# ICLDisco/parsec

Measured on AMD Instinct MI355X. Metric: GFLOP/s (whole node) tiled Cholesky N=80k, higher is better.
Workload: dtype fp64; 1 GPU; model=tiled_cholesky_dpotrf, N=80000, tile=4096, parallelism=dtd-tile-p1q1, chore_gemm=rocblas, gpu=True

## Files before the change

### src/kernels_hip.cpp

```cpp
#include "kernels_hip.hpp"

#include "kernels.hpp"

namespace pa {

typedef double f64x4 __attribute__((ext_vector_type(4)));

#define BM 128
#define BN 128
#define BKD 16


__device__ __forceinline__ int xcd_swizzle(int id, int nwg) {
  int q = nwg >> 3, r = nwg & 7;
  int xcd = id & 7, pos = id >> 3;
  return (xcd < r ? xcd * (q + 1) : r * (q + 1) + (xcd - r) * q) + pos;
}

__device__ __forceinline__ void tri_decode(int id, int& i, int& j) {
  i = 0;
  while (id > i) { i++; id -= i; }
  j = id;
}

__device__ __forceinline__ void block_decode(bool tri, int nbx, int& bx,
                                             int& by) {
  int id = xcd_swizzle(blockIdx.x, gridDim.x);
  if (tri) {
    tri_decode(id, bx, by);
  } else {
    bx = id % nbx;
    by = id / nbx;
  }
}

__device__ __forceinline__ void mfma_ktile(f64x4 (&acc)[2][4],
                                           const double* ap, const double* bp,
                                           int ld) {
#pragma unroll
  for (int kk = 0; kk < BKD; kk += 4) {
    double a[2], b[4];
#pragma unroll
    for (int f = 0; f < 2; f++) a[f] = ap[kk * ld + f * 16];
#pragma unroll
    for (int f = 0; f < 4; f++) b[f] = bp[kk * ld + f * 16];
#pragma unroll
    for (int i = 0; i < 2; i++)
#pragma unroll
      for (int j = 0; j < 4; j++)
        acc[i][j] =
            __builtin_amdgcn_mfma_f64_16x16x4f64(a[i], b[j], acc[i][j], 0, 0, 0);
  }
}

__device__ __forceinline__ void write_c(const f64x4 (&acc)[2][4], double* C,
                                        int ldc, int row0, int col0, int m,
                                        int n, bool checked, bool store) {
#pragma unroll
  for (int j = 0; j < 4; j++) {
    int col = col0 + j * 16;
    if (checked && col >= n) continue;
    double* cp = C + (size_t)col * ldc;
#pragma unroll
    for (int i = 0; i < 2; i++) {
#pragma unroll
      for (int e = 0; e < 4; e++) {
        int row = row0 + i * 16 + e * 4;
        if (checked && row >= m) continue;
        if (store) cp[row] = acc[i][j][e];
        else cp[row] -= acc[i][j][e];
      }
    }
  }
}

template <bool TRI>
__launch_bounds__(512)
__global__ void k_dgemm_nt_v2(int m, int n, int k, const double* __restrict__ A,
                              int lda, const double* __restrict__ B, int ldb,
                              double* __restrict__ C, int ldc, int nbx) {
  extern __shared__ __attribute__((aligned(16))) char smem[];
  constexpr int LDT = 129;
  double* As = (double*)smem;
  double* Bs = As + 2 * BKD * LDT;
  const int tid = threadIdx.x;
  const int wave = tid >> 6, lane = tid & 63;
  const int wr = wave >> 1, wc = wave & 1;
  int bx, by;
  block_decode(TRI, nbx, bx, by);
  const int bm0 = bx * BM, bn0 = by * BN;
  const int ksub = lane >> 4, r16 = lane & 15;

  f64x4 acc[2][4] = {};

  auto stage = [&](int buf, int k0) {
    double* as = As + buf * BKD * LDT;
    double* bs = Bs + buf * BKD * LDT;
#pragma unroll
    for (int x = 0; x < BM * BKD; x += 512) {
      int xi = x + tid;
      int i = xi & (BM - 1), kk = xi >> 7;
      int gi = bm0 + i, gk = k0 + kk;
      as[kk * LDT + i] = (gi < m && gk < k) ? A[(size_t)gk * lda + gi] : 0.0;
    }
#pragma unroll
    for (int x = 0; x < BN * BKD; x += 512) {
      int xi = x + tid;
      int j = xi & (BN - 1), kk = xi >> 7;
      int gj = bn0 + j, gk = k0 + kk;
      bs[kk * LDT + j] = (gj < n && gk < k) ? B[(size_t)gk * ldb + gj] : 0.0;
    }
  };

  stage(0, 0);
  __syncthreads();
  const int ntiles = (k + BKD - 1) / BKD;
  for (int t = 0; t < ntiles; t++) {
    if (t + 1 < ntiles) stage((t + 1) & 1, (t + 1) * BKD);
    mfma_ktile(acc, As + ((t & 1) * BKD + ksub) * LDT + wr * 32 + r16,
               Bs + ((t & 1) * BKD + ksub) * LDT + wc * 64 + r16, LDT);
    __syncthreads();
  }
  write_c(acc, C, ldc, bm0 + wr * 32 + ksub, bn0 + wc * 64 + r16, m, n,
          true, false);
}

enum { V3_GEMM = 0, V3_SYRK = 1, V3_TRMM = 2 };

template <int KIND>
__launch_bounds__(512)
__global__ void k_dgemm_nt_v3(int m, int n, int k, const double* __restrict__ A,
                              int lda, const double* __restrict__ B, int ldb,
                              double* __restrict__ C, int ldc, int nbx) {
  extern __shared__ __attribute__((aligned(16))) char smem[];
  double* As = (double*)smem;
  double* Bs = As + 2 * BKD * BM;
  const int tid = threadIdx.x;
  const int wave = tid >> 6, lane = tid & 63;
  const int wr = wave >> 1, wc = wave & 1;
  int bx, by;
  if (KIND == V3_TRMM) {
    const int nby = n / BN;
    const int xcd = blockIdx.x & 7, pos = blockIdx.x >> 3;
    const int round = pos / nbx;
    const int rank = round * 8 + ((round & 1) ? 7 - xcd : xcd);
    if (rank >= nby) return;
    bx = pos - round * nbx;
    by = nby - 1 - rank;
  } else {
    block_decode(KIND == V3_SYRK, nbx, bx, by);
  }
  const int bm0 = bx * BM, bn0 = by * BN;
  const int ksub = lane >> 4, r16 = lane & 15;
  const int kend = KIND == V3_TRMM ? (bn0 + BN < k ? bn0 + BN : k) : k;

  f64x4 acc[2][4] = {};

  auto stage = [&](int buf, int k0) {
#pragma unroll
    for (int p = 0; p < 2; p++) {
      int krow = wave * 2 + p;
      const double* srcA = A + (size_t)(k0 + krow) * lda + bm0 + 2 * lane;
      double* dstA = As + buf * BKD * BM + krow * BM;
      __builtin_amdgcn_global_load_lds(
          (const __attribute__((address_space(1))) unsigned int*)srcA,
          (__attribute__((address_space(3))) unsigned int*)dstA, 16, 0, 0);
      const double* srcB = B + (size_t)(k0 + krow) * ldb + bn0 + 2 * lane;
      double* dstB = Bs + buf * BKD * BN + krow * BN;
      __builtin_amdgcn_global_load_lds(
          (const __attribute__((address_space(1))) unsigned int*)srcB,
          (__attribute__((address_space(3))) unsigned int*)dstB, 16, 0, 0);
    }
  };

  stage(0, 0);
  __syncthreads();
  const int ntiles = kend / BKD;
  for (int t = 0; t < ntiles; t++) {
    if (t + 1 < ntiles) stage((t + 1) & 1, (t + 1) * BKD);
    mfma_ktile(acc, As + ((t & 1) * BKD + ksub) * BM + wr * 32 + r16,
               Bs + ((t & 1) * BKD + ksub) * BN + wc * 64 + r16, BM);
    __syncthreads();
  }
  write_c(acc, C, ldc, bm0 + wr * 32 + ksub, bn0 + wc * 64 + r16, m, n,
          false, KIND == V3_TRMM);
}

template <auto Kern, typename... Args>
static void launch_lds(int grid, int block, size_t lds, hipStream_t stream,
                       Args... args) {
  static const bool raised = [lds] {
    PA_HIP_CHECK(hipFuncSetAttribute(
        (const void*)Kern, hipFuncAttributeMaxDynamicSharedMemorySize, lds));
    return true;
  }();
  (void)raised;
  hipLaunchKernelGGL(Kern, dim3(grid), dim3(block), lds, stream, args...);
}

constexpr size_t LDS_V2 = 4 * BKD * 129 * 8;
constexpr size_t LDS_V3 = 2 * BKD * (BM + BN) * 8;

static bool full_tiles(int m, int n, int k, int lda, int ldb) {
  return m % BM == 0 && n % BN == 0 && k % BKD == 0 && lda % 2 == 0 &&
         ldb % 2 == 0;
}

void launch_dgemm_nt(int m, int n, int k, const double* A, int lda,
                     const double* B, int ldb, double* C, int ldc,
                     hipStream_t stream) {
  const int nbx = (m + BM - 1) / BM, nby = (n + BN - 1) / BN;
  if (full_tiles(m, n, k, lda, ldb))
    launch_lds<k_dgemm_nt_v3<V3_GEMM>>(nbx * nby, 512, LDS_V3, stream, m, n, k,
                                       A, lda, B, ldb, C, ldc, nbx);
  else
    launch_lds<k_dgemm_nt_v2<false>>(nbx * nby, 512, LDS_V2, stream, m, n, k,
                                     A, lda, B, ldb, C, ldc, nbx);
}

void launch_dsyrk_ln(int n, int k, const double* A, int lda, double* C,
                     int ldc, hipStream_t stream) {
  const int ntb = (n + BM - 1) / BM;
  const int nblocks = ntb * (ntb + 1) / 2;
  if (full_tiles(n, n, k, lda, lda))
    launch_lds<k_dgemm_nt_v3<V3_SYRK>>(nblocks, 512, LDS_V3, stream, n, n, k,
                                       A, lda, A, lda, C, ldc, 0);
  else
    launch_lds<k_dgemm_nt_v2<true>>(nblocks, 512, LDS_V2, stream, n, n, k, A,
                                    lda, A, lda, C, ldc, 0);
}

void launch_dtrmm_rlt(int m, int n, const double* B, int ldb, const double* W,
                      int ldw, double* X, int ldx, hipStream_t stream) {
  PA_CHECK(m > 0 && n > 0 && full_tiles(m, n, n, ldb, ldw),
           "dtrmm_rlt needs full 128x128 blocks and even ld, got %d x %d, "
           "ldb %d, ldw %d", m, n, ldb, ldw);
  PA_CHECK(ldb >= m && ldx >= m && ldw >= n);
  const int nbx = m / BM, nby = n / BN;
  launch_lds<k_dgemm_nt_v3<V3_TRMM>>(8 * ((nby + 7) / 8) * nbx, 512, LDS_V3,
                                     stream, m, n, n, B, ldb, W, ldw, X, ldx,
                                     nbx);
}

void gpu_gemm_hip(Task& t, GpuTaskCtx& g) {
  const TileArgs& a = t.arg<TileArgs>();
  launch_dgemm_nt(a.m, a.n, a.k, (const double*)t.dev_ptr[0], a.ld,
                  (const double*)t.dev_ptr[1], a.ld, (double*)t.dev_ptr[2],
                  a.ld, g.stream);
}

__global__ void __launch_bounds__(256) k_potf2_mfma(double* A, int n, int ld) {
  extern __shared__ __attribute__((aligned(16))) char smem[];
  constexpr int LDP = 129;
  double* S = (double*)smem;
  double* dinv = S + 128 * LDP;
  const int tid = threadIdx.x;
  const int lane = tid & 63;
  const int wave = tid >> 6;
  for (int x = tid; x < n * n; x += 256) {
    int j = x / n, i = x - j * n;
    if (i >= j) S[j * LDP + i] = A[(size_t)j * ld + i];
  }
  __syncthreads();
  for (int jb = 0; jb < n; jb += 16) {
    const int jbe = jb + 16 < n ? jb + 16 : n;
    for (int j = jb; j < jbe; j++) {
      if (tid == 0) {
        double d = S[j * LDP + j];
        S[j * LDP + j] = d = sqrt(d);
        *dinv = 1.0 / d;
      }
      __syncthreads();
      for (int i = j + 1 + tid; i < n; i += 256) S[j * LDP + i] *= *dinv;
      __syncthreads();
      for (int c = j + 1 + wave; c < jbe; c += 4) {
        double ljc = S[j * LDP + c];
        for (int i = c + lane; i < n; i += 64)
          S[c * LDP + i] -= S[j * LDP + i] * ljc;
      }
      __syncthreads();
    }
    const int t0 = jbe;
    const int nt = (n - t0 + 15) >> 4;
    if (nt > 0) {
      const int ntiles = nt * (nt + 1) / 2;
      const int r16 = lane & 15, g4 = lane >> 4;
      for (int idx = wave; idx < ntiles; idx += 4) {
        int ti, tj;
        tri_decode(idx, ti, tj);
        const int ro = t0 + ti * 16, co = t0 + tj * 16;
        const int arow = ro + r16, brow = co + r16;
        f64x4 acc;
#pragma unroll
        for (int e = 0; e < 4; e++) {
          int r = ro + 4 * e + g4, c = co + r16;
          acc[e] = (r < n && c < n) ? S[c * LDP + r] : 0.0;
        }
#pragma unroll
        for (int kk = 0; kk < 16; kk += 4) {
          int kcol = jb + kk + g4;
          double a = (arow < n) ? -S[kcol * LDP + arow] : 0.0;
          double b = (brow < n) ? S[kcol * LDP + brow] : 0.0;
          acc = __builtin_amdgcn_mfma_f64_16x16x4f64(a, b, acc, 0, 0, 0);
        }
#pragma unroll
        for (int e = 0; e < 4; e++) {
          int r = ro + 4 * e + g4, c = co + r16;
          if (r < n && c < n && r >= c) S[c * LDP + r] = acc[e];
        }
      }
    }
    __syncthreads();
  }
  for (int x = tid; x < n * n; x += 256) {
    int j = x / n, i = x - j * n;
    if (i >= j) A[(size_t)j * ld + i] = S[j * LDP + i];
  }
}

void launch_potf2(double* A, int n, int ld, hipStream_t stream) {
  PA_CHECK(n <= 128);
  launch_lds<k_potf2_mfma>(1, 256, 128 * 129 * 8 + 16, stream, A, n, ld);
}

namespace {

struct DevArray {
  double* p = nullptr;
  size_t bytes;
  explicit DevArray(size_t nelem, const double* host = nullptr)
      : bytes(nelem * 8) {
    PA_HIP_CHECK(hipMalloc(&p, bytes));
    if (host) PA_HIP_CHECK(hipMemcpy(p, host, bytes, hipMemcpyHostToDevice));
  }
  DevArray(const DevArray&) = delete;
  ~DevArray() { PA_HIP_CHECK(hipFree(p)); }
  void download(double* host) {
    PA_HIP_CHECK(hipGetLastError());
    PA_HIP_CHECK(hipMemcpy(host, p, bytes, hipMemcpyDeviceToHost));
  }
};

__global__ void k_bench_fill(double* p, size_t n, uint32_t seed) {
  size_t i = (size_t)blockIdx.x * blockDim.x + threadIdx.x;
  for (; i < n; i += (size_t)gridDim.x * blockDim.x) {
    uint64_t h = (i * 2654435761ull) ^ ((uint64_t)seed * 2246822519ull);
    h ^= h >> 13;
    h *= 0x9E3779B97F4A7C15ull;
    h ^= h >> 32;
    p[i] = (double)(h & 0xFFFFFF) / (double)0x1000000 - 0.5;
  }
}

void bench_fill(DevArray& a, uint32_t seed) {
  hipLaunchKernelGGL(k_bench_fill, dim3(2048), dim3(256), 0, 0, a.p,
                     a.bytes / 8, seed);
}

template <typename F>
double time_launches(int iters, F run) {
  run();
  PA_HIP_CHECK(hipDeviceSynchronize());
  double t0 = now_s();
  for (int i = 0; i < iters; i++) run();
  PA_HIP_CHECK(hipDeviceSynchronize());
  return now_s() - t0;
}

}

void test_dgemm_nt_hip(int m, int n, int k, const double* A, int lda,
                       const double* B, int ldb, double* C, int ldc) {
  DevArray dA((size_t)lda * k, A), dB((size_t)ldb * k, B),
      dC((size_t)ldc * n, C);
  launch_dgemm_nt(m, n, k, dA.p, lda, dB.p, ldb, dC.p, ldc, 0);
  dC.download(C);
}

void test_dsyrk_ln_hip(int n, int k, const double* A, int lda, double* C,
                       int ldc) {
  DevArray dA((size_t)lda * k, A), dC((size_t)ldc * n, C);
  launch_dsyrk_ln(n, k, dA.p, lda, dC.p, ldc, 0);
  dC.download(C);
}

void test_dtrmm_rlt_hip(int m, int n, const double* B, int ldb,
                        const double* W, int ldw, double* X, int ldx) {
  DevArray dB((size_t)ldb * n, B), dW((size_t)ldw * n, W),
      dX((size_t)ldx * n, X);
  launch_dtrmm_rlt(m, n, dB.p, ldb, dW.p, ldw, dX.p, ldx, 0);
  dX.download(X);
}

void test_potf2_hip(double* A, int n) {
  DevArray dA((size_t)n * n, A);
  launch_potf2(dA.p, n, n, 0);
  dA.download(A);
}

double bench_dgemm_hip(int m, int n, int k, int iters) {
  DevArray dA((size_t)m * k), dB((size_t)n * k), dC((size_t)m * n);
  bench_fill(dA, 11);
  bench_fill(dB, 12);
  bench_fill(dC, 13);
  return time_launches(iters, [&] {
    launch_dgemm_nt(m, n, k, dA.p, m, dB.p, n, dC.p, m, 0);
  });
}

double bench_dtrmm_hip(int m, int n, int iters) {
  DevArray dB((size_t)m * n), dW((size_t)n * n), dX((size_t)m * n);
  bench_fill(dB, 11);
  bench_fill(dW, 12);
  for (int c = 1; c < n; c++)
    PA_HIP_CHECK(hipMemsetAsync(dW.p + (size_t)c * n, 0, (size_t)c * 8, 0));
  return time_launches(iters, [&] {
    launch_dtrmm_rlt(m, n, dB.p, m, dW.p, n, dX.p, m, 0);
  });
}

}
```

### src/kernels_hip.hpp

```cpp
#pragma once

#include "device_gpu.hpp"

namespace pa {

void launch_dgemm_nt(int m, int n, int k, const double* A, int lda,
                     const double* B, int ldb, double* C, int ldc,
                     hipStream_t stream);
void launch_dsyrk_ln(int n, int k, const double* A, int lda, double* C,
                     int ldc, hipStream_t stream);
void launch_dtrmm_rlt(int m, int n, const double* B, int ldb, const double* W,
                      int ldw, double* X, int ldx, hipStream_t stream);
void launch_potf2(double* A, int n, int ld, hipStream_t stream);

void gpu_gemm_hip(Task& t, GpuTaskCtx& g);

void test_dgemm_nt_hip(int m, int n, int k, const double* A, int lda,
                       const double* B, int ldb, double* C, int ldc);
void test_dsyrk_ln_hip(int n, int k, const double* A, int lda, double* C,
                       int ldc);
void test_dtrmm_rlt_hip(int m, int n, const double* B, int ldb,
                        const double* W, int ldw, double* X, int ldx);
void test_potf2_hip(double* A, int n);

double bench_dgemm_hip(int m, int n, int k, int iters);
double bench_dtrmm_hip(int m, int n, int iters);

}
```

### src/pybind.cpp

```cpp
#include <pybind11/numpy.h>
#include <pybind11/pybind11.h>
#include <pybind11/stl.h>

#include <chrono>
#include <map>

#include "data.hpp"
#include "device_gpu.hpp"
#include "comm.hpp"
#include "dtd.hpp"
#include "gpu_graph.hpp"
#include "kernels.hpp"
#include "kernels_hip.hpp"
#include "pins.hpp"
#include "profiling.hpp"
#include "runtime.hpp"

namespace pa {
std::string rccl_get_unique_id();
void rccl_set_unique_id(const std::string&);
double bench_dgemm_rocblas(int, int, int, int);
double bench_gemm_bf16(int, int, int, int);
double bench_qr_factor(int, int, int, int, int);
void test_gemm_bf16_hip(int, int, int, const uint16_t*, const uint16_t*,
                        float*);
}

namespace py = pybind11;
using namespace pa;

namespace {

struct PyTaskPayload {
  PyObject* fn;
  int with_data;
};

void py_task_hook(Task& t) {
  const PyTaskPayload& pl = t.arg<PyTaskPayload>();
  void* bufs[MAX_FLOWS] = {};
  if (pl.with_data) {
    for (int i = 0; i < t.nflows; i++) {
      Data* d = t.flows[i].data;
      if (!d) continue;
      if (t.flows[i].mode & ACCESS_IN) {
        bufs[i] = d->pull_to_host();
      } else {
        d->begin_host_overwrite();
        bufs[i] = d->ensure_host();
      }
    }
  }
  py::gil_scoped_acquire gil;
  py::handle fn(pl.fn);
  try {
    if (pl.with_data) {
      py::tuple args(t.nflows);
      for (int i = 0; i < t.nflows; i++) {
        Data* d = t.flows[i].data;
        if (d)
          args[i] = py::memoryview::from_memory(bufs[i], (ssize_t)d->bytes);
        else
          args[i] = py::none();
      }
      fn(*args);
    } else {
      fn();
    }
  } catch (py::error_already_set& e) {
    fprintf(stderr, "[parsec_amd] python task raised: %s\n", e.what());
  }
  for (int i = 0; i < t.nflows && pl.with_data; i++)
    if (t.flows[i].data && (t.flows[i].mode & ACCESS_OUT))
      t.flows[i].data->written_on(false);
}

void py_task_destruct(Task& t) {
  py::gil_scoped_acquire gil;
  Py_XDECREF(t.arg<PyTaskPayload>().fn);
}

TaskClass& py_task_class() {
  static TaskClass tc = [] {
    TaskClass c;
    c.name = "py_task";
    c.kind = TaskKind::CPU;
    c.cpu_hook = py_task_hook;
    c.destruct = py_task_destruct;
    c.id = 100;
    return c;
  }();
  return tc;
}

Context::Options options_from_env(int nworkers, int rank, int world,
                                  std::string comm, int gpu) {
  Context::Options o;
  o.nworkers = nworkers;
  if (rank < 0) {
    const char* r = getenv("RANK");
    const char* w = getenv("WORLD_SIZE");
    o.rank = r ? atoi(r) : 0;
    o.world = w ? atoi(w) : 1;
  } else {
    o.rank = rank;
    o.world = world;
  }
  o.comm = std::move(comm);
  o.gpu_device = gpu;
  return o;
}

}

PYBIND11_MODULE(_core, m) {
  m.doc() = "parsec_amd: MI355X-native task-dataflow runtime (PaRSEC-class)";

  py::class_<Context>(m, "Context")
      .def(py::init([](int nworkers, int rank, int world, std::string comm,
                       int gpu) {
             return new Context(
                 options_from_env(nworkers, rank, world, std::move(comm), gpu));
           }),
           py::arg("nworkers") = -1, py::arg("rank") = -1,
           py::arg("world") = -1, py::arg("comm") = std::string(),
           py::arg("gpu") = -1,
           py::call_guard<py::gil_scoped_release>())
      .def_property_readonly("_handle", [](Context& c) { return (uintptr_t)&c; })
      .def_property_readonly("rank", &Context::rank)
      .def_property_readonly("world", &Context::world)
      .def_property_readonly("nworkers", &Context::nworkers)
      .def_property_readonly("has_gpu", &Context::has_gpu)
      .def("barrier", &Context::barrier,
           py::call_guard<py::gil_scoped_release>())
      .def("gpu_sync", [](Context& c) {
        if (c.gpu()) c.gpu()->sync_all();
      }, py::call_guard<py::gil_scoped_release>())
      .def("gpu_stats", [](Context& c) {
        py::dict d;
        if (c.gpu()) {
          d["tasks"] = c.gpu()->stats.tasks.load();
          d["bytes_h2d"] = c.gpu()->stats.bytes_h2d.load();
          d["bytes_d2h"] = c.gpu()->stats.bytes_d2h.load();
          d["evictions"] = c.gpu()->stats.evictions.load();
          d["bytes_required"] = c.gpu()->stats.bytes_required.load();
        }
        return d;
      })
      .def("send_ctl", [](Context& c, int dst, uint32_t tag, py::bytes b) {
        PA_CHECK(c.comm(), "send_ctl: no comm engine");
        std::string s(b);
        py::gil_scoped_release rel;
        c.comm()->send_ctl(dst, tag, s.data(), s.size());
      }, py::arg("dst"), py::arg("tag"), py::arg("payload"))
      .def("set_ctl_handler", [](Context& c, py::function fn) {
        PA_CHECK(c.comm(), "set_ctl_handler: no comm engine");
        PyObject* f = fn.ptr();
        Py_XINCREF(f);
        c.comm()->set_ctl_handler(
            [f](int src, uint32_t tag, const std::string& pl) {
              py::gil_scoped_acquire gil;
              try {
                py::handle h(f);
                h(src, tag, py::bytes(pl));
              } catch (py::error_already_set& e) {
                fprintf(stderr, "[parsec_amd] ctl handler raised: %s\n",
                        e.what());
              }
            });
      })
      .def("info", [](Context& c) {
        py::dict d;
        for (auto& [k, v] : c.info_all()) d[py::str(k)] = v;
        return d;
      })
      .def("info_set", [](Context& c, std::string k, std::string v) {
        c.info_set(k, v);
      })
      .def("comm_stats", [](Context& c) {
        py::list out;
        if (c.comm()) {
          for (auto& ps : c.comm()->peer_stats()) {
            py::dict d;
            d["sent_msgs"] = ps.sent_msgs.load();
            d["sent_bytes"] = ps.sent_bytes.load();
            d["recv_msgs"] = ps.recv_msgs.load();
            d["recv_bytes"] = ps.recv_bytes.load();
            out.append(d);
          }
        }
        return out;
      })
      .def("counters", [](Context&) {
        auto& c = counters();
        py::dict d;
        d["tasks_executed_cpu"] = c.tasks_executed_cpu.load();
        d["tasks_executed_gpu"] = c.tasks_executed_gpu.load();
        d["tasks_scheduled"] = c.tasks_scheduled.load();
        d["steals"] = c.steals.load();
        d["comm_msgs"] = c.comm_msgs.load();
        d["comm_bytes"] = c.comm_bytes.load();
        d["renames"] = c.renames.load();
        return d;
      });

  py::class_<Data>(m, "Data")
      .def_property_readonly("home_rank", [](Data& d) { return d.home_rank; })
      .def_property_readonly("owner_rank", [](Data& d) { return d.owner_rank; })
      .def_property_readonly("version", [](Data& d) { return d.version; })
      .def_property_readonly("nbytes", [](Data& d) { return d.bytes; });

  py::class_<TiledMatrix>(m, "TiledMatrix")
      .def(py::init<Context*, int64_t, int64_t, int, int, int, int, size_t,
                    bool>(),
           py::arg("ctx"), py::arg("m"), py::arg("n"), py::arg("mb"),
           py::arg("nb"), py::arg("p") = 1, py::arg("q") = 1,
           py::arg("elem_size") = 8, py::arg("sym") = false,
           py::keep_alive<1, 2>())
      .def_property_readonly("_handle", [](TiledMatrix& a) { return (uintptr_t)&a; })
      .def_property_readonly("m", &TiledMatrix::m)
      .def_property_readonly("n", &TiledMatrix::n)
      .def_property_readonly("mt", &TiledMatrix::mt)
      .def_property_readonly("nt", &TiledMatrix::nt)
      .def_property_readonly("mb", &TiledMatrix::mb)
      .def_property_readonly("nb", &TiledMatrix::nb)
      .def("rank_of", &TiledMatrix::rank_of)
      .def("set_kcyclic", &TiledMatrix::set_kcyclic)
      .def("set_rank_table", &TiledMatrix::set_rank_table)
      .def("set_band", &TiledMatrix::set_band)
      .def("in_band", &TiledMatrix::in_band)
      .def("is_local", &TiledMatrix::is_local)
      .def("tile", &TiledMatrix::tile, py::return_value_policy::reference_internal)
      .def("tile_rows", &TiledMatrix::tile_rows)
      .def("tile_cols", &TiledMatrix::tile_cols)
      .def("tile_numpy", [](TiledMatrix& A, int tm, int tn) {
        PA_CHECK(A.is_local(tm, tn), "tile_numpy: tile is not local");
        Data* d = A.tile(tm, tn);
        double* p;
        {
          py::gil_scoped_release rel;
          p = (double*)d->pull_to_host();
        }
        int rows = A.tile_rows(tm), cols = A.tile_cols(tn);
        py::array_t<double> out({rows, cols});
        auto r = out.mutable_unchecked<2>();
        for (int j = 0; j < cols; j++)
          for (int i = 0; i < rows; i++) r(i, j) = p[(size_t)j * A.mb() + i];
        return out;
      })
      .def("tile_numpy_set", [](TiledMatrix& A, int tm, int tn,
                                py::array_t<double> v) {
        PA_CHECK(A.is_local(tm, tn), "tile_numpy_set: tile is not local");
        Data* d = A.tile(tm, tn);
        d->begin_host_overwrite();
        double* p = (double*)d->ensure_host();
        auto r = v.unchecked<2>();
        int rows = A.tile_rows(tm), cols = A.tile_cols(tn);
        PA_CHECK(r.shape(0) == rows && r.shape(1) == cols);
        for (int j = 0; j < cols; j++)
          for (int i = 0; i < rows; i++) p[(size_t)j * A.mb() + i] = r(i, j);
        d->written_on(false);
      })
      .def("tile_bytes", [](TiledMatrix& A, int tm, int tn) {
        PA_CHECK(A.is_local(tm, tn));
        Data* d = A.tile(tm, tn);
        void* p;
        {
          py::gil_scoped_release rel;
          p = d->pull_to_host();
        }
        return py::bytes((const char*)p, d->bytes);
      })
      .def("tile_bytes_set", [](TiledMatrix& A, int tm, int tn, py::bytes b) {
        PA_CHECK(A.is_local(tm, tn));
        Data* d = A.tile(tm, tn);
        d->begin_host_overwrite();
        std::string s(b);
        PA_CHECK(s.size() <= d->bytes);
        memcpy(d->ensure_host(), s.data(), s.size());
        d->written_on(false);
      });

  py::class_<ZoneAlloc>(m, "ZoneAlloc")
      .def(py::init([](size_t bytes) {
             auto* z = new ZoneAlloc();
             z->init(bytes);
             return z;
           }),
           py::arg("bytes"))
      .def("alloc",
           [](ZoneAlloc& z, size_t sz) -> py::object {
             size_t off = z.alloc(sz);
             if (off == ZoneAlloc::NPOS) return py::none();
             return py::int_(off);
           })
      .def("free", &ZoneAlloc::free, py::arg("off"), py::arg("size"))
      .def_property_readonly("in_use", &ZoneAlloc::in_use)
      .def_property_readonly("capacity", &ZoneAlloc::capacity)
      .def_property_readonly("largest_free", &ZoneAlloc::largest_free)
      .def_property_readonly("free_blocks", &ZoneAlloc::free_blocks);

  py::class_<IrregularCollection>(m, "IrregularCollection")
      .def(py::init<Context*>(), py::arg("ctx"), py::keep_alive<1, 2>())
      .def("add", &IrregularCollection::add, py::arg("key"), py::arg("rank"),
           py::arg("bytes"), py::return_value_policy::reference_internal)
      .def("at", &IrregularCollection::at, py::arg("key"),
           py::return_value_policy::reference_internal)
      .def_property_readonly("size", &IrregularCollection::size)
      .def("bytes_get", [](IrregularCollection& c, uint64_t key) {
        Data* d = c.at(key);
        void* p;
        {
          py::gil_scoped_release rel;
          p = d->pull_to_host();
        }
        return py::bytes((const char*)p, d->bytes);
      })
      .def("bytes_set", [](IrregularCollection& c, uint64_t key, py::bytes b) {
        Data* d = c.at(key);
        d->begin_host_overwrite();
        std::string s2(b);
        PA_CHECK(s2.size() <= d->bytes);
        memcpy(d->ensure_host(), s2.data(), s2.size());
        d->written_on(false);
      });

  py::class_<Taskpool>(m, "Taskpool")
      .def("wait_dynamic", &Taskpool::wait_dynamic,
           py::call_guard<py::gil_scoped_release>())
      .def_property_readonly("_handle", [](Taskpool& t) { return (uintptr_t)&t; })
      .def("wait", &Taskpool::wait, py::call_guard<py::gil_scoped_release>())
      .def_property_readonly("pending", &Taskpool::pending)
      .def("on_complete", [](Taskpool& t, py::function fn) {
        auto holder = std::shared_ptr<py::function>(
            new py::function(std::move(fn)), [](py::function* p) {
              py::gil_scoped_acquire gil;
              delete p;
            });
        t.on_complete([holder] {
          py::gil_scoped_acquire gil;
          try {
            (*holder)();
          } catch (py::error_already_set& e) {
            fprintf(stderr, "[parsec_amd] on_complete raised: %s\n", e.what());
          }
        });
      });

  py::class_<Dtd, Taskpool>(m, "Dtd")
      .def(py::init<Context*, std::string>(), py::arg("ctx"),
           py::arg("name") = std::string("dtd"), py::keep_alive<1, 2>())
      .def("insert_py",
           [](Dtd& tp, py::function fn, py::list flows, int priority,
              int rank, bool with_data) {
             PyTaskPayload pl{fn.ptr(), with_data ? 1 : 0};
             Py_XINCREF(pl.fn);
             std::vector<Dtd::FlowSpec> fs;
             for (auto h : flows) {
               auto t2 = h.cast<py::tuple>();
               Dtd::FlowSpec f{t2[0].cast<Data*>(),
                               (AccessMode)t2[1].cast<int>(),
                               Reshape::NONE};
               if (t2.size() > 2) f.reshape = (Reshape)t2[2].cast<int>();
               fs.push_back(f);
             }
             bool local;
             {
               py::gil_scoped_release rel;
               local = tp.insert(&py_task_class(), &pl, sizeof(pl),
                                 fs.data(), (int)fs.size(), priority, rank);
             }
             if (!local) Py_XDECREF(pl.fn);
           },
           py::arg("fn"), py::arg("flows") = py::list(),
           py::arg("priority") = 0, py::arg("rank") = -1,
           py::arg("with_data") = false)
      .def("flush", &Dtd::flush, py::call_guard<py::gil_scoped_release>())
      .def("flush_all", &Dtd::flush_all,
           py::call_guard<py::gil_scoped_release>())
      .def("capture_begin", &Dtd::capture_begin)
      .def("capture_end", &Dtd::capture_end,
           py::call_guard<py::gil_scoped_release>(),
           py::keep_alive<0, 1>());

  py::class_<GpuGraph>(m, "GpuGraph")
      .def("launch", &GpuGraph::launch, py::arg("iters") = 1,
           py::call_guard<py::gil_scoped_release>())
      .def_property_readonly("nodes", &GpuGraph::nodes)
      .def_property_readonly("n_tasks", &GpuGraph::n_tasks);

  m.attr("ACCESS_IN") = (int)ACCESS_IN;
  m.attr("ACCESS_UNTRACKED") = (int)ACCESS_UNTRACKED;
  m.attr("ACCESS_OUT") = (int)ACCESS_OUT;
  m.attr("ACCESS_INOUT") = (int)ACCESS_INOUT;
  m.attr("RESHAPE_TRANSPOSE") = (int)Reshape::TRANSPOSE;
  m.attr("RESHAPE_TO_BF16") = (int)Reshape::TO_BF16;
  m.attr("RESHAPE_FROM_BF16") = (int)Reshape::FROM_BF16;
  m.attr("RESHAPE_TRIL") = (int)Reshape::TRIL;
  m.attr("RESHAPE_TRIU") = (int)Reshape::TRIU;

  m.def("bench_qr_factor", &bench_qr_factor, py::arg("m"), py::arg("k"),
        py::arg("ts_split"), py::arg("iters"), py::arg("mode"),
        py::call_guard<py::gil_scoped_release>());
  m.def("insert_spd_fill", &insert_spd_fill, py::arg("tp"), py::arg("A"),
        py::arg("seed") = 42u, py::call_guard<py::gil_scoped_release>());
  m.def("insert_full_fill", &insert_full_fill, py::arg("tp"), py::arg("A"),
        py::arg("seed") = 42u, py::call_guard<py::gil_scoped_release>());
  m.def("insert_potrf", &insert_potrf, py::arg("tp"), py::arg("A"),
        py::call_guard<py::gil_scoped_release>());
  m.def("insert_getrf_nopiv", &insert_getrf_nopiv, py::arg("tp"),
        py::arg("A"), py::call_guard<py::gil_scoped_release>());
  m.def("insert_geqrf", &insert_geqrf, py::arg("tp"), py::arg("A"),
        py::call_guard<py::gil_scoped_release>());
  m.def("insert_geqrf_bcgs", &insert_geqrf_bcgs, py::arg("tp"),
        py::arg("A"), py::arg("R"), py::call_guard<py::gil_scoped_release>());
  m.def("insert_redistribute", &insert_redistribute, py::arg("tp"),
        py::arg("src"), py::arg("dst"), py::call_guard<py::gil_scoped_release>());
  m.def("insert_reduce_axis", &insert_reduce_axis, py::arg("tp"),
        py::arg("A"), py::arg("R"), py::arg("axis"),
        py::call_guard<py::gil_scoped_release>());
  m.def("insert_band_to_rect", &insert_band_to_rect, py::arg("tp"),
        py::arg("S"), py::arg("D"), py::call_guard<py::gil_scoped_release>());
  m.def("insert_subtile_extract", &insert_subtile_extract, py::arg("tp"),
        py::arg("A"), py::arg("tm"), py::arg("tn"), py::arg("S"),
        py::call_guard<py::gil_scoped_release>());
  m.def("insert_subtile_insert", &insert_subtile_insert, py::arg("tp"),
        py::arg("S"), py::arg("A"), py::arg("tm"), py::arg("tn"),
        py::call_guard<py::gil_scoped_release>());
  m.def("insert_potrs", &insert_potrs, py::arg("tp"), py::arg("A"),
        py::arg("B"), py::call_guard<py::gil_scoped_release>());
  m.def("insert_posv", &insert_posv, py::arg("tp"), py::arg("A"),
        py::arg("B"), py::call_guard<py::gil_scoped_release>());
  m.def("insert_getrs_nopiv", &insert_getrs_nopiv, py::arg("tp"),
        py::arg("A"), py::arg("B"), py::call_guard<py::gil_scoped_release>());
  m.def("insert_gesv_nopiv", &insert_gesv_nopiv, py::arg("tp"),
        py::arg("A"), py::arg("B"), py::call_guard<py::gil_scoped_release>());
  m.def("insert_gels_bcgs", &insert_gels_bcgs, py::arg("tp"), py::arg("A"),
        py::arg("R"), py::arg("B"), py::arg("X"),
        py::call_guard<py::gil_scoped_release>());
  m.def("insert_advise_prefetch", &insert_advise_prefetch, py::arg("tp"),
        py::arg("tile"), py::call_guard<py::gil_scoped_release>());
  m.def("insert_gemm_fp64", &insert_gemm_fp64, py::arg("tp"), py::arg("A"),
        py::arg("B"), py::arg("C"),
        py::call_guard<py::gil_scoped_release>());
  m.def("insert_apply_scale", &insert_apply_scale, py::arg("tp"), py::arg("A"),
        py::arg("alpha"), py::arg("beta"),
        py::call_guard<py::gil_scoped_release>());
  m.def("insert_reduce_sum_tree", &insert_reduce_sum_tree, py::arg("tp"),
        py::arg("A"), py::arg("R"), py::call_guard<py::gil_scoped_release>());
  m.def("insert_reduce_sum", &insert_reduce_sum, py::arg("tp"), py::arg("A"),
        py::arg("R"), py::call_guard<py::gil_scoped_release>());
  m.def("insert_stencil_1d", &insert_stencil_1d, py::arg("tp"),
        py::arg("src"), py::arg("dst"), py::call_guard<py::gil_scoped_release>());
  m.def("insert_panel_fill", &insert_panel_fill, py::arg("tp"), py::arg("A"),
        py::arg("seed") = 42u, py::call_guard<py::gil_scoped_release>());
  m.def("insert_potrf_panel", &insert_potrf_panel, py::arg("tp"),
        py::arg("A"), py::call_guard<py::gil_scoped_release>());
  m.def("insert_fill_bf16", &insert_fill_bf16, py::arg("tp"), py::arg("A"),
        py::arg("seed") = 1u, py::call_guard<py::gil_scoped_release>());
  m.def("insert_gemm_bf16", &insert_gemm_bf16, py::arg("tp"), py::arg("At"),
        py::arg("B"), py::arg("C"), py::call_guard<py::gil_scoped_release>());
  m.def("bench_gemm_bf16", [](int m, int n, int k, int iters) {
    return pa::bench_gemm_bf16(m, n, k, iters);
  }, py::call_guard<py::gil_scoped_release>());
  m.def("gemm_bf16_hip", [](py::array_t<uint16_t> A, py::array_t<uint16_t> B,
                            py::array_t<float> C, int m, int n, int k) {
    pa::test_gemm_bf16_hip(m, n, k, A.data(), B.data(), C.mutable_data());
  });

  m.def("pins_add", [](py::function fn, std::vector<std::string> events) {
    static const std::map<std::string, PinsEv> names = {
        {"exec_begin", PinsEv::EXEC_BEGIN}, {"exec_end", PinsEv::EXEC_END},
        {"schedule", PinsEv::SCHEDULE},     {"complete", PinsEv::COMPLETE},
        {"gpu_submit", PinsEv::GPU_SUBMIT}, {"gpu_retire", PinsEv::GPU_RETIRE},
        {"create", PinsEv::CREATE},
        {"release_deps", PinsEv::RELEASE_DEPS},
        {"stage_in", PinsEv::STAGE_IN},     {"comm_post", PinsEv::COMM_POST},
        {"comm_done", PinsEv::COMM_DONE},   {"steal", PinsEv::STEAL}};
    uint32_t mask = 0;
    for (auto& e : events) {
      auto it = names.find(e);
      if (it == names.end())
        throw std::invalid_argument("unknown PINS event: " + e);
      mask |= 1u << (int)it->second;
    }
    auto keep = std::shared_ptr<py::function>(
        new py::function(std::move(fn)), [](py::function* f) {
          py::gil_scoped_acquire g;
          delete f;
        });
    static const char* evname[] = {"exec_begin", "exec_end",   "schedule",
                                   "complete",   "gpu_submit", "gpu_retire",
                                   "create",     "release_deps", "stage_in",
                                   "comm_post",  "comm_done",  "steal"};
    return Pins::inst().add(
        [keep](PinsEv e, const Task* t, int worker) {
          py::gil_scoped_acquire g;
          (*keep)(evname[(int)e], t ? t->tc->name : std::string(), worker);
        },
        mask);
  });
  m.def("pins_remove", [](int id) { Pins::inst().remove(id); });

  m.def("set_fatal_handler", [](py::function fn) {
    static py::function* g_fn = nullptr;
    if (g_fn) { delete g_fn; }
    g_fn = new py::function(std::move(fn));
    set_fatal_handler(+[](const char* msg) {
      py::gil_scoped_acquire g;
      try { (*reinterpret_cast<py::function*>(g_fn))(msg); } catch (...) {}
    });
  });

  m.def("param_set", &param_set);
  m.def("param_dump", &param_dump);
  m.def("hip_device_count", [] {
    int n = 0;
    if (hipGetDeviceCount(&n) != hipSuccess) n = 0;
    return n;
  });
  m.def("dgemm_nt_hip", [](py::array_t<double> A, py::array_t<double> B,
                           py::array_t<double> C, int m, int n, int k, int lda,
                           int ldb, int ldc) {
    if (lda == 0) lda = m;
    if (ldb == 0) ldb = n;
    if (ldc == 0) ldc = m;
    if (m <= 0 || n <= 0 || k <= 0 || lda < m || ldb < n || ldc < m ||
        A.size() < (py::ssize_t)lda * k || B.size() < (py::ssize_t)ldb * k ||
        C.size() < (py::ssize_t)ldc * n)
      throw std::invalid_argument("dgemm_nt_hip: buffer smaller than ld*cols");
    pa::test_dgemm_nt_hip(m, n, k, A.data(), lda, B.data(), ldb,
                          C.mutable_data(), ldc);
  }, py::arg("A"), py::arg("B"), py::arg("C"), py::arg("m"), py::arg("n"),
     py::arg("k"), py::arg("lda") = 0, py::arg("ldb") = 0, py::arg("ldc") = 0);
  m.def("dsyrk_ln_hip", [](py::array_t<double> A, py::array_t<double> C, int n,
                           int k, int lda, int ldc) {
    if (n <= 0 || k <= 0 || lda < n || ldc < n ||
        A.size() < (py::ssize_t)lda * k || C.size() < (py::ssize_t)ldc * n)
      throw std::invalid_argument("dsyrk_ln_hip: buffer smaller than ld*cols");
    pa::test_dsyrk_ln_hip(n, k, A.data(), lda, C.mutable_data(), ldc);
  });
  m.def("dtrmm_rlt_hip", [](py::array_t<double> B, py::array_t<double> W,
                            py::array_t<double> X, int m, int n, int ldb,
                            int ldw, int ldx) {
    if (m <= 0 || n <= 0 || ldb < m || ldx < m || ldw < n ||
        B.size() < (py::ssize_t)ldb * n || W.size() < (py::ssize_t)ldw * n ||
        X.size() < (py::ssize_t)ldx * n)
      throw std::invalid_argument("dtrmm_rlt_hip: buffer smaller than ld*n");
    pa::test_dtrmm_rlt_hip(m, n, B.data(), ldb, W.data(), ldw,
                           X.mutable_data(), ldx);
  });
  m.def("potf2_hip", [](py::array_t<double> A, int n) {
    pa::test_potf2_hip(A.mutable_data(), n);
  });
  m.def("bench_dtrmm", [](int m, int n, int iters) {
    return pa::bench_dtrmm_hip(m, n, iters) / iters * 1e3;
  }, py::call_guard<py::gil_scoped_release>());
  m.def("bench_dgemm", [](int m, int n, int k, int iters, std::string impl) {
    if (impl != "hip" && impl != "v2" && impl != "rocblas")
      throw std::invalid_argument("bench_dgemm: impl is \"hip\" or \"rocblas\"");
    double dt = impl == "rocblas" ? pa::bench_dgemm_rocblas(m, n, k, iters)
                                  : pa::bench_dgemm_hip(m, n, k, iters);
    return 2.0 * m * n * k * iters / dt / 1e12;
  }, py::call_guard<py::gil_scoped_release>());
  m.def("hip_bandwidth", [](size_t nbytes, int iters) {
    void *hbuf = nullptr, *d0 = nullptr, *d1 = nullptr;
    if (hipHostMalloc(&hbuf, nbytes) != hipSuccess)
      throw std::runtime_error("hipHostMalloc failed");
    if (hipMalloc(&d0, nbytes) != hipSuccess ||
        hipMalloc(&d1, nbytes) != hipSuccess)
      throw std::runtime_error("hipMalloc failed");
    hipStream_t s;
    (void)hipStreamCreate(&s);
    auto run = [&](void* dst, const void* src, hipMemcpyKind kind) {
      (void)hipMemcpyAsync(dst, src, nbytes, kind, s);
      (void)hipStreamSynchronize(s);
      auto t0 = std::chrono::steady_clock::now();
      for (int i = 0; i < iters; i++)
        (void)hipMemcpyAsync(dst, src, nbytes, kind, s);
      (void)hipStreamSynchronize(s);
      double dt = std::chrono::duration<double>(
                      std::chrono::steady_clock::now() - t0).count();
      return (double)nbytes * iters / dt / 1e9;
    };
    py::dict r;
    r["h2d_gbs"] = run(d0, hbuf, hipMemcpyHostToDevice);
    r["d2h_gbs"] = run(hbuf, d0, hipMemcpyDeviceToHost);
    r["d2d_gbs"] = run(d1, d0, hipMemcpyDeviceToDevice);
    r["bytes"] = nbytes;
    (void)hipStreamDestroy(s);
    (void)hipFree(d0);
    (void)hipFree(d1);
    (void)hipHostFree(hbuf);
    return r;
  }, py::arg("nbytes") = (size_t)256 << 20, py::arg("iters") = 20);
  m.def("nccl_unique_id", [] { return py::bytes(pa::rccl_get_unique_id()); });
  m.def("set_nccl_unique_id",
        [](py::bytes b) { pa::rccl_set_unique_id(std::string(b)); });
}
```

Baseline: 67020 GFLOP/s.

## Rework v3 GEMM kernel into a 4-stage LDS ring with fine-grained vmcnt waits

Replaces the double-buffered v3 kernel with a 4-stage LDS ring of smaller K-tiles. Async global-to-LDS loads are issued several tiles ahead and waited on with explicit vmcnt counts, using one barrier per tile. LDS fragments are read via inline asm with immediate offsets, and launch bounds ask for 2 blocks per CU. This aims to hide memory latency and cut per-tile synchronisation and address arithmetic for the GEMM, SYRK and TRMM paths, at the cost of hand-written waitcnt asm that is fragile. A dsyrk benchmark binding is also added.

Result: no change. 66980 GFLOP/s (-0.1%).

```diff
diff --git a/src/kernels_hip.cpp b/src/kernels_hip.cpp
--- a/src/kernels_hip.cpp
+++ b/src/kernels_hip.cpp
@@ -34,18 +34,19 @@
   }
 }
 
-__device__ __forceinline__ void mfma_ktile(f64x4 (&acc)[2][4],
+template <int BK, int FM>
+__device__ __forceinline__ void mfma_ktile(f64x4 (&acc)[FM][4],
                                            const double* ap, const double* bp,
                                            int ld) {
 #pragma unroll
-  for (int kk = 0; kk < BKD; kk += 4) {
-    double a[2], b[4];
-#pragma unroll
-    for (int f = 0; f < 2; f++) a[f] = ap[kk * ld + f * 16];
+  for (int kk = 0; kk < BK; kk += 4) {
+    double a[FM], b[4];
+#pragma unroll
+    for (int f = 0; f < FM; f++) a[f] = ap[kk * ld + f * 16];
 #pragma unroll
     for (int f = 0; f < 4; f++) b[f] = bp[kk * ld + f * 16];
 #pragma unroll
-    for (int i = 0; i < 2; i++)
+    for (int i = 0; i < FM; i++)
 #pragma unroll
       for (int j = 0; j < 4; j++)
         acc[i][j] =
@@ -53,7 +54,43 @@
   }
 }
 
-__device__ __forceinline__ void write_c(const f64x4 (&acc)[2][4], double* C,
+__device__ __forceinline__ double lds_read_imm(unsigned addr, int off) {
+  double v;
+  asm volatile("ds_read_b64 %0, %1 offset:%2" : "=v"(v) : "v"(addr), "n"(off));
+  return v;
+}
+template <int BK, int FM>
+__device__ __forceinline__ void mfma_ktile_imm(f64x4 (&acc)[FM][4],
+                                               unsigned aaddr, unsigned baddr,
+                                               int off) {
+#pragma unroll
+  for (int kk = 0; kk < BK; kk += 4) {
+    double a[FM], b[4];
+#pragma unroll
+    for (int f = 0; f < FM; f++)
+      a[f] = lds_read_imm(aaddr, off + (kk * BM + f * 16) * 8);
+#pragma unroll
+    for (int f = 0; f < 4; f++)
+      b[f] = lds_read_imm(baddr, off + (kk * BM + f * 16) * 8);
+    if constexpr (FM == 2)
+      asm volatile("s_waitcnt lgkmcnt(0)"
+                   : "+v"(a[0]), "+v"(a[1]), "+v"(b[0]), "+v"(b[1]),
+                     "+v"(b[2]), "+v"(b[3]));
+    else
+      asm volatile("s_waitcnt lgkmcnt(0)"
+                   : "+v"(a[0]), "+v"(a[1]), "+v"(a[2]), "+v"(a[3]),
+                     "+v"(b[0]), "+v"(b[1]), "+v"(b[2]), "+v"(b[3]));
+#pragma unroll
+    for (int i = 0; i < FM; i++)
+#pragma unroll
+      for (int j = 0; j < 4; j++)
+        acc[i][j] =
+            __builtin_amdgcn_mfma_f64_16x16x4f64(a[i], b[j], acc[i][j], 0, 0, 0);
+  }
+}
+
+template <int FM>
+__device__ __forceinline__ void write_c(const f64x4 (&acc)[FM][4], double* C,
                                         int ldc, int row0, int col0, int m,
                                         int n, bool checked, bool store) {
 #pragma unroll
@@ -62,7 +99,7 @@
     if (checked && col >= n) continue;
     double* cp = C + (size_t)col * ldc;
 #pragma unroll
-    for (int i = 0; i < 2; i++) {
+    for (int i = 0; i < FM; i++) {
 #pragma unroll
       for (int e = 0; e < 4; e++) {
         int row = row0 + i * 16 + e * 4;
@@ -117,8 +154,8 @@
   const int ntiles = (k + BKD - 1) / BKD;
   for (int t = 0; t < ntiles; t++) {
     if (t + 1 < ntiles) stage((t + 1) & 1, (t + 1) * BKD);
-    mfma_ktile(acc, As + ((t & 1) * BKD + ksub) * LDT + wr * 32 + r16,
-               Bs + ((t & 1) * BKD + ksub) * LDT + wc * 64 + r16, LDT);
+    mfma_ktile<BKD, 2>(acc, As + ((t & 1) * BKD + ksub) * LDT + wr * 32 + r16,
+                       Bs + ((t & 1) * BKD + ksub) * LDT + wc * 64 + r16, LDT);
     __syncthreads();
   }
   write_c(acc, C, ldc, bm0 + wr * 32 + ksub, bn0 + wc * 64 + r16, m, n,
@@ -127,16 +164,38 @@
 
 enum { V3_GEMM = 0, V3_SYRK = 1, V3_TRMM = 2 };
 
+template <int N>
+__device__ __forceinline__ void wait_vmcnt() {
+  asm volatile("s_waitcnt vmcnt(%0)" ::"n"(N) : "memory");
+}
+
+template <int G, int R>
+__device__ __forceinline__ void wait_tiles_ahead(int ahead) {
+  if constexpr (R == 0) {
+    wait_vmcnt<0>();
+  } else {
+    if (ahead >= R) wait_vmcnt<G * R>();
+    else wait_tiles_ahead<G, R - 1>(ahead);
+  }
+}
+
+constexpr int V3_NW = 8, V3_S = 4, V3_BK = 8;
+
 template <int KIND>
-__launch_bounds__(512)
+__launch_bounds__(V3_NW * 64, 2)
 __global__ void k_dgemm_nt_v3(int m, int n, int k, const double* __restrict__ A,
                               int lda, const double* __restrict__ B, int ldb,
                               double* __restrict__ C, int ldc, int nbx) {
+  constexpr int NW = V3_NW, S = V3_S, BK = V3_BK;
+  static_assert(S >= 3 && BK % 4 == 0 && BK % NW == 0 && BM == BN);
+  constexpr int FM = 16 / NW;
+  constexpr int APW = BK / NW;
+  constexpr int G = 2 * APW;
+  constexpr int STAGE = 2 * BK * BM;
   extern __shared__ __attribute__((aligned(16))) char smem[];
-  double* As = (double*)smem;
-  double* Bs = As + 2 * BKD * BM;
+  double* ring = (double*)smem;
   const int tid = threadIdx.x;
-  const int wave = tid >> 6, lane = tid & 63;
+  const int wave = __builtin_amdgcn_readfirstlane(tid >> 6), lane = tid & 63;
   const int wr = wave >> 1, wc = wave & 1;
   int bx, by;
   if (KIND == V3_TRMM) {
@@ -154,36 +213,61 @@
   const int ksub = lane >> 4, r16 = lane & 15;
   const int kend = KIND == V3_TRMM ? (bn0 + BN < k ? bn0 + BN : k) : k;
 
-  f64x4 acc[2][4] = {};
-
+  f64x4 acc[FM][4] = {};
+
+  const char* rowA = (const char*)(A + (size_t)wave * lda + bm0);
+  const char* rowB = (const char*)(B + (size_t)wave * ldb + bn0);
+  const unsigned lane16 = lane * 16;
+  auto uniform = [](const char* p) {
+    size_t v = (size_t)p;
+    unsigned lo = __builtin_amdgcn_readfirstlane((unsigned)v);
+    unsigned hi = __builtin_amdgcn_readfirstlane((unsigned)(v >> 32));
+    return (const char*)(((size_t)hi << 32) | lo);
+  };
   auto stage = [&](int buf, int k0) {
-#pragma unroll
-    for (int p = 0; p < 2; p++) {
-      int krow = wave * 2 + p;
-      const double* srcA = A + (size_t)(k0 + krow) * lda + bm0 + 2 * lane;
-      double* dstA = As + buf * BKD * BM + krow * BM;
+    double* dst = ring + buf * STAGE + wave * BM;
+#pragma unroll
+    for (int p = 0; p < APW; p++) {
       __builtin_amdgcn_global_load_lds(
-          (const __attribute__((address_space(1))) unsigned int*)srcA,
-          (__attribute__((address_space(3))) unsigned int*)dstA, 16, 0, 0);
-      const double* srcB = B + (size_t)(k0 + krow) * ldb + bn0 + 2 * lane;
-      double* dstB = Bs + buf * BKD * BN + krow * BN;
+          (const __attribute__((address_space(1))) unsigned int*)(
+              uniform(rowA + (size_t)(k0 + p * NW) * lda * 8) + lane16),
+          (__attribute__((address_space(3))) unsigned int*)(dst + p * NW * BM),
+          16, 0, 0);
+    }
+#pragma unroll
+    for (int p = 0; p < APW; p++) {
       __builtin_amdgcn_global_load_lds(
-          (const __attribute__((address_space(1))) unsigned int*)srcB,
-          (__attribute__((address_space(3))) unsigned int*)dstB, 16, 0, 0);
+          (const __attribute__((address_space(1))) unsigned int*)(
+              uniform(rowB + (size_t)(k0 + p * NW) * ldb * 8) + lane16),
+          (__attribute__((address_space(3))) unsigned int*)(
+              dst + (BK + p * NW) * BM),
+          16, 0, 0);
     }
   };
 
-  stage(0, 0);
-  __syncthreads();
-  const int ntiles = kend / BKD;
-  for (int t = 0; t < ntiles; t++) {
-    if (t + 1 < ntiles) stage((t + 1) & 1, (t + 1) * BKD);
-    mfma_ktile(acc, As + ((t & 1) * BKD + ksub) * BM + wr * 32 + r16,
-               Bs + ((t & 1) * BKD + ksub) * BN + wc * 64 + r16, BM);
-    __syncthreads();
-  }
-  write_c(acc, C, ldc, bm0 + wr * 32 + ksub, bn0 + wc * 64 + r16, m, n,
-          false, KIND == V3_TRMM);
+  const int ntiles = kend / BK;
+#pragma unroll
+  for (int s = 0; s < S - 1; s++)
+    if (s < ntiles) stage(s, s * BK);
+  static_assert(S * STAGE * 8 <= 65536, "stage offsets are 16-bit immediates");
+  const unsigned rd = (unsigned)(size_t)(
+      (__attribute__((address_space(3))) double*)ring) + (ksub * BM + r16) * 8;
+  const unsigned rda = rd + wr * (16 * FM) * 8;
+  const unsigned rdb = rd + (BK * BM + wc * 64) * 8;
+  for (int t0 = 0; t0 < ntiles; t0 += S) {
+#pragma unroll
+    for (int s = 0; s < S; s++) {
+      const int t = t0 + s;
+      if (t >= ntiles) break;
+      wait_tiles_ahead<G, S - 2>(ntiles - 1 - t);
+      asm volatile("s_waitcnt lgkmcnt(0)" ::: "memory");
+      __builtin_amdgcn_s_barrier();
+      if (t + S - 1 < ntiles) stage((s + S - 1) % S, (t + S - 1) * BK);
+      mfma_ktile_imm<BK, FM>(acc, rda, rdb, s * STAGE * 8);
+    }
+  }
+  write_c<FM>(acc, C, ldc, bm0 + wr * (16 * FM) + ksub, bn0 + wc * 64 + r16, m,
+              n, false, KIND == V3_TRMM);
 }
 
 template <auto Kern, typename... Args>
@@ -199,10 +283,11 @@
 }
 
 constexpr size_t LDS_V2 = 4 * BKD * 129 * 8;
-constexpr size_t LDS_V3 = 2 * BKD * (BM + BN) * 8;
+
+constexpr size_t LDS_V3 = (size_t)V3_S * 2 * V3_BK * BM * 8;
 
 static bool full_tiles(int m, int n, int k, int lda, int ldb) {
-  return m % BM == 0 && n % BN == 0 && k % BKD == 0 && lda % 2 == 0 &&
+  return m % BM == 0 && n % BN == 0 && k % V3_BK == 0 && lda % 2 == 0 &&
          ldb % 2 == 0;
 }
 
@@ -211,8 +296,8 @@
                      hipStream_t stream) {
   const int nbx = (m + BM - 1) / BM, nby = (n + BN - 1) / BN;
   if (full_tiles(m, n, k, lda, ldb))
-    launch_lds<k_dgemm_nt_v3<V3_GEMM>>(nbx * nby, 512, LDS_V3, stream, m, n, k,
-                                       A, lda, B, ldb, C, ldc, nbx);
+    launch_lds<k_dgemm_nt_v3<V3_GEMM>>(nbx * nby, V3_NW * 64, LDS_V3, stream, m,
+                                       n, k, A, lda, B, ldb, C, ldc, nbx);
   else
     launch_lds<k_dgemm_nt_v2<false>>(nbx * nby, 512, LDS_V2, stream, m, n, k,
                                      A, lda, B, ldb, C, ldc, nbx);
@@ -223,8 +308,8 @@
   const int ntb = (n + BM - 1) / BM;
   const int nblocks = ntb * (ntb + 1) / 2;
   if (full_tiles(n, n, k, lda, lda))
-    launch_lds<k_dgemm_nt_v3<V3_SYRK>>(nblocks, 512, LDS_V3, stream, n, n, k,
-                                       A, lda, A, lda, C, ldc, 0);
+    launch_lds<k_dgemm_nt_v3<V3_SYRK>>(nblocks, V3_NW * 64, LDS_V3, stream, n,
+                                       n, k, A, lda, A, lda, C, ldc, 0);
   else
     launch_lds<k_dgemm_nt_v2<true>>(nblocks, 512, LDS_V2, stream, n, n, k, A,
                                     lda, A, lda, C, ldc, 0);
@@ -237,9 +322,9 @@
            "ldb %d, ldw %d", m, n, ldb, ldw);
   PA_CHECK(ldb >= m && ldx >= m && ldw >= n);
   const int nbx = m / BM, nby = n / BN;
-  launch_lds<k_dgemm_nt_v3<V3_TRMM>>(8 * ((nby + 7) / 8) * nbx, 512, LDS_V3,
-                                     stream, m, n, n, B, ldb, W, ldw, X, ldx,
-                                     nbx);
+  launch_lds<k_dgemm_nt_v3<V3_TRMM>>(8 * ((nby + 7) / 8) * nbx, V3_NW * 64,
+                                     LDS_V3, stream, m, n, n, B, ldb, W, ldw,
+                                     X, ldx, nbx);
 }
 
 void gpu_gemm_hip(Task& t, GpuTaskCtx& g) {
@@ -408,6 +493,15 @@
   });
 }
 
+double bench_dsyrk_hip(int n, int k, int iters) {
+  DevArray dA((size_t)n * k), dC((size_t)n * n);
+  bench_fill(dA, 11);
+  bench_fill(dC, 13);
+  return time_launches(iters, [&] {
+    launch_dsyrk_ln(n, k, dA.p, n, dC.p, n, 0);
+  });
+}
+
 double bench_dtrmm_hip(int m, int n, int iters) {
   DevArray dB((size_t)m * n), dW((size_t)n * n), dX((size_t)m * n);
   bench_fill(dB, 11);
diff --git a/src/kernels_hip.hpp b/src/kernels_hip.hpp
--- a/src/kernels_hip.hpp
+++ b/src/kernels_hip.hpp
@@ -25,5 +25,6 @@
 
 double bench_dgemm_hip(int m, int n, int k, int iters);
 double bench_dtrmm_hip(int m, int n, int iters);
+double bench_dsyrk_hip(int n, int k, int iters);
 
 }
diff --git a/src/pybind.cpp b/src/pybind.cpp
--- a/src/pybind.cpp
+++ b/src/pybind.cpp
@@ -556,6 +556,9 @@
   m.def("bench_dtrmm", [](int m, int n, int iters) {
     return pa::bench_dtrmm_hip(m, n, iters) / iters * 1e3;
   }, py::call_guard<py::gil_scoped_release>());
+  m.def("bench_dsyrk", [](int n, int k, int iters) {
+    return pa::bench_dsyrk_hip(n, k, iters) / iters * 1e3;
+  }, py::call_guard<py::gil_scoped_release>());
   m.def("bench_dgemm", [](int m, int n, int k, int iters, std::string impl) {
     if (impl != "hip" && impl != "v2" && impl != "rocblas")
       throw std::invalid_argument("bench_dgemm: impl is \"hip\" or \"rocblas\"");
```
